# matpalm/cartpoleplusplus

Hardware: AMD Instinct MI355X
Metric: DDPG training steps/sec, 64x64x18 pixel obs, batch=256 (higher is better)
Workload: dtype f32-acc/f16x2,bf16x6

## Files before the change

cartpoleplusplus_amd/csrc/conv3_bwd_pair.hip:

```cpp
#include <cstring>
#ifndef PAIR_ORDER_DEFAULT
#define PAIR_ORDER_DEFAULT 1
#endif
#include "conv_impl.h"
#include "conv_kyo.h"
#include "conv_dx_rs.h"
#include "conv_dw_rs.h"

__global__ __launch_bounds__(CONV_THREADS, 2) void conv3_bwd_pair_kernel(const ConvArgsN dx, int dx_gx, const ConvArgsN dw, int dw_gx, int order) {
  int i;
  if (!pair_grid_place((int)blockIdx.x, dx_gx * dx.n, dw_gx * dw.n, order, &i)) {
    conv_fwd_kyo_body<10, 3, 1, 4, IN_DY, 16, false>(dx, i % dx_gx, i / dx_gx);
  } else {
    conv_dw_body<10, 3, 1, IN_F32_PLAIN>(dw, i % dw_gx, i / dw_gx, dw_gx);
  }
}

template <int ORDER>
__global__ __launch_bounds__(CONV_THREADS, 2) __attribute__((amdgpu_waves_per_eu(2, 2))) void conv3_bwd_pair_rs_kernel(const ConvArgsN dx, int dx_gx, const ConvArgsN dw, int dw_gx, int upi, int band, int order) {
  int i;
  if (!pair_grid_place((int)blockIdx.x, dx_gx * dx.n, dw_gx * dw.n, order, &i)) {
    conv_dx_rs_body<3, 1, ORDER>(dx, i % dx_gx, i / dx_gx);
  } else {
    conv_dw_rs_body<3, ORDER>(dw, upi, band, i % dw_gx, i / dw_gx);
  }
}

template <int ORDER, bool DXRS>
__global__ __launch_bounds__(CONV_THREADS, 2) void conv3_bwd_pair_mixed_kernel(const ConvArgsN dx, int dx_gx, const ConvArgsN dw, int dw_gx, int upi, int band, int order) {
  int i;
  if (!pair_grid_place((int)blockIdx.x, dx_gx * dx.n, dw_gx * dw.n, order, &i)) {
    if (DXRS) conv_dx_rs_body<3, 1, ORDER>(dx, i % dx_gx, i / dx_gx);
    else conv_fwd_kyo_body<10, 3, 1, 4, IN_DY, 16, false>(dx, i % dx_gx, i / dx_gx);
  } else {
    if (DXRS) conv_dw_body<10, 3, 1, IN_F32_PLAIN>(dw, i % dw_gx, i / dw_gx, dw_gx);
    else conv_dw_rs_body<3, ORDER>(dw, upi, band, i % dw_gx, i / dw_gx);
  }
}

int launch_conv3_bwd_pair(cpp_ctx* ctx, const ConvPairSlot& slot) {
  const bool dx_rs = slot.have_dx && slot.dx_rs, dw_rs = slot.have_dw && slot.dw_rs;
  if (slot.have_dx && slot.have_dw && dx_rs != dw_rs) {
    const bool nine = b16_order(ctx) == B16_NINE;
    auto kern = dx_rs ? (nine ? conv3_bwd_pair_mixed_kernel<B16_NINE, true> : conv3_bwd_pair_mixed_kernel<B16_SIX, true>)
                      : (nine ? conv3_bwd_pair_mixed_kernel<B16_NINE, false> : conv3_bwd_pair_mixed_kernel<B16_SIX, false>);
    const size_t lds = slot.dx_lds > slot.dw_lds ? slot.dx_lds : slot.dw_lds;
    HIP_CHECK(hipFuncSetAttribute((const void*)kern, hipFuncAttributeMaxDynamicSharedMemorySize, (int)lds));
    static const int order = cpp_switch_int("CPP_PAIR3_ORDER", 1);
    prof_begin(ctx);
    hipLaunchKernelGGL(kern, dim3(slot.dx_gx * slot.dx.n + slot.dw_gx * slot.dw.n), dim3(CONV_THREADS), lds, ctx->stream, slot.dx, slot.dx_gx, slot.dw, slot.dw_gx,
                       slot.upi, slot.band, order);
    LAUNCH_CHECK();
    prof_end(ctx, K_CONV3_BWD);
    return 0;
  }
  if (dx_rs || dw_rs) {
    if (!(dx_rs && dw_rs)) { cpp_set_error("conv3 backward pair: one half is missing beside a row-streaming body"); return 1; }
    const bool nine = b16_order(ctx) == B16_NINE;
    auto kern = nine ? conv3_bwd_pair_rs_kernel<B16_NINE> : conv3_bwd_pair_rs_kernel<B16_SIX>;
    const size_t lds = slot.dx_lds > slot.dw_lds ? slot.dx_lds : slot.dw_lds;
    static bool attr_done[CPP_MAX_DEVICES][2] = {};
    if (!attr_done[cpp_dev_slot(ctx)][nine ? 1 : 0]) {
      HIP_CHECK(hipFuncSetAttribute((const void*)kern, hipFuncAttributeMaxDynamicSharedMemorySize, (int)lds));
      attr_done[cpp_dev_slot(ctx)][nine ? 1 : 0] = true;
    }
    static const int order = cpp_switch_int("CPP_PAIR3_ORDER", 1);
    prof_begin(ctx);
    hipLaunchKernelGGL(kern, dim3(slot.dx_gx * slot.dx.n + slot.dw_gx * slot.dw.n), dim3(CONV_THREADS), lds, ctx->stream, slot.dx, slot.dx_gx, slot.dw, slot.dw_gx,
                       slot.upi, slot.band, order);
    LAUNCH_CHECK();
    prof_end(ctx, K_CONV3_BWD);
    return 0;
  }
  const int ndx = slot.have_dx ? slot.dx_gx * slot.dx.n : 0, ndw = slot.have_dw ? slot.dw_gx * slot.dw.n : 0;
  if (ndx + ndw == 0) return 0;
  const size_t lds = (slot.have_dx ? slot.dx_lds : 0) > (slot.have_dw ? slot.dw_lds : 0) ? slot.dx_lds : slot.dw_lds;
  static size_t attr_dev[CPP_MAX_DEVICES] = {};
  size_t& attr = attr_dev[cpp_dev_slot(ctx)];
  if (lds > attr) {
    HIP_CHECK(hipFuncSetAttribute((const void*)conv3_bwd_pair_kernel, hipFuncAttributeMaxDynamicSharedMemorySize, (int)lds));
    attr = lds;
  }
  ConvArgsN dx = slot.dx, dw = slot.dw;
  if (!slot.have_dx) { memset(&dx, 0, sizeof(dx)); dx.n = 0; }
  if (!slot.have_dw) { memset(&dw, 0, sizeof(dw)); dw.n = 0; }
  static const int order = cpp_switch_int("CPP_PAIR_ORDER", PAIR_ORDER_DEFAULT);
  prof_begin(ctx);
  hipLaunchKernelGGL(conv3_bwd_pair_kernel, dim3(ndx + ndw), dim3(CONV_THREADS), lds, ctx->stream, dx, slot.have_dx ? slot.dx_gx : 1,
                     dw, slot.have_dw ? slot.dw_gx : 1, order);
  LAUNCH_CHECK();
  prof_end(ctx, K_CONV3_BWD);
  return 0;
}
```

cartpoleplusplus_amd/csrc/conv_dw_rs.hip:

```cpp
#include <cstring>
#include "conv_dw_rs.h"

int conv_dw_rs_dispatch(cpp_ctx* ctx, int cin, int ks, int in_mode, const ConvArgsN& batch, int* grid_out, bool* handled) {
  *handled = false;
  static const bool off = cpp_switch_off("CPP_CONV_DWRS") || cpp_switch_off("CPP_CONV_B16");
  const ConvArgs& a = batch.a[0];
  static const bool off3 = cpp_switch_off("CPP_CONV3_DWRS");
  static const bool w16 = cpp_switch_int("CPP_CONV3_DWRS_W16", 0) != 0;
  const bool geo5 = ks == 5 && (a.W == 32 || a.W == 64), geo3 = ks == 3 && !off3 && ((a.W == 16 && (w16 || conv3_pair_rs_ok(ctx, a.H, a.W))) || a.W == 32 || a.W == 64);
  if (off || !(geo5 || geo3) || cin != KYO_NO || in_mode != IN_F32_PLAIN || (a.H & 1) || a.H < 8 || a.nout != KYO_NO) return 0;
  for (int i = 0; i < batch.n; ++i)
    if (batch.a[i].dy_dense != nullptr || ((uintptr_t)batch.a[i].in & 7) || (batch.a[i].in_bstride & 1)) return 0;
  *handled = true;
  const int capacity = ctx->num_cus * 4 / batch.n, ncol = (a.W + 31) / 32;
  int band = (a.H + 1) & ~1;
  while (band > 8 && (band / 2) % 2 == 0 && a.B * ncol * ((a.H + band / 2 - 1) / (band / 2)) <= capacity) band /= 2;
  const int upi = ((a.H + band - 1) / band) * ncol;
  const int grid = (a.B * upi + 3) / 4;
  if ((size_t)grid > (size_t)ctx->num_cus * 4) { *handled = false; return 0; }
  *grid_out = grid;
  const bool nine = b16_order(ctx) == B16_NINE;
  if (ctx->pair && ctx->pair->layer == 1 && ks == 5 && a.W == 32) {
    ctx->pair->dw = batch; ctx->pair->dw_gx = grid; ctx->pair->dw_lds = DwRsGeom<5>::LDS_BYTES; ctx->pair->have_dw = true;
    ctx->pair->upi = upi; ctx->pair->band = band; ctx->pair->dw_rs = true;
    return 0;
  }
  if (ks == 3 && conv3_pair_rs_ok(ctx, a.H, a.W)) {
    ctx->pair->dw = batch; ctx->pair->dw_gx = grid; ctx->pair->dw_lds = DwRsGeom<3>::LDS_BYTES; ctx->pair->have_dw = true;
    ctx->pair->upi = upi; ctx->pair->band = band; ctx->pair->dw_rs = true;
    return 0;
  }
  typedef void (*kern_t)(const ConvArgsN, int, int);
  const kern_t kern = ks == 5 ? (nine ? (kern_t)conv_dw_rs_kernel<5, B16_NINE> : (kern_t)conv_dw_rs_kernel<5, B16_SIX>)
                              : (nine ? (kern_t)conv_dw_rs_kernel<3, B16_NINE> : (kern_t)conv_dw_rs_kernel<3, B16_SIX>);
  const int lds = ks == 5 ? DwRsGeom<5>::LDS_BYTES : DwRsGeom<3>::LDS_BYTES;
  static bool attr_done[CPP_MAX_DEVICES][4] = {};
  bool& done = attr_done[cpp_dev_slot(ctx)][(nine ? 1 : 0) + (ks == 5 ? 0 : 2)];
  if (!done) {
    HIP_CHECK(hipFuncSetAttribute((const void*)kern, hipFuncAttributeMaxDynamicSharedMemorySize, lds));
    done = true;
  }
  hipLaunchKernelGGL(kern, dim3(grid, batch.n), dim3(CONV_THREADS), lds, ctx->stream, batch, upi, band);
  LAUNCH_CHECK();
  return 0;
}
```

cartpoleplusplus_amd/csrc/conv_dx_rs.h:

```cpp
#pragma once
#include <type_traits>
#include "conv_k16.h"

typedef unsigned dxrs_u32x2 __attribute__((ext_vector_type(2)));

template <int KS_, int TPR>
struct DxRsGeom {
  static constexpr int KS = KS_, P = KS / 2, CH = KYO_NO, NCH = (KS * CH + 31) / 32, NSET = KS + 1;
  static constexpr int UNR = KS == 5 ? 6 : 12;
  static constexpr int W = 16 * TPR, IPW = 4 / TPR;
  static constexpr int NW = KS * KS * CH * CH;
  static constexpr int AIMG_BYTES = KS * NCH * 3 * 1024;
  static constexpr int WPX = 16 + 2 * P;
  static constexpr int PLB = ((2 * CH * 15 + 64 * (NCH - 1) + 64 + 15) & ~15) + 16;
  static constexpr int SLOTB = 3 * PLB;
  static constexpr int TRB = 640 + 16;
  static constexpr int WVB = 2 * SLOTB + TRB;
  static constexpr int LDS_BYTES = AIMG_BYTES + 4 * WVB;
  static_assert((KS == 5 || KS == 3) && 4 % TPR == 0 && WVB % 16 == 0 && PLB >= 2 * CH * WPX + 8, "geometry");
};

template <int KSZ, int TPR, int ORDER>
__device__ __forceinline__ void conv_dx_rs_body(const ConvArgsN& batch, const int bx, const int by) {
  typedef DxRsGeom<KSZ, TPR> G;
  constexpr int KS = G::KS, P = G::P, CH = G::CH, NCH = G::NCH, NSET = G::NSET, UNR = G::UNR, W = G::W, Wp = W / 2;
  constexpr int PLB = G::PLB, SLOTB = G::SLOTB;
  const ConvArgs& a = batch.a[by];
  extern __shared__ __attribute__((aligned(16))) unsigned char dxrs_lds[];
  const int tid = threadIdx.x, lane = tid & 63, li = lane & 15, lj = lane >> 4;
  const int swave = __builtin_amdgcn_readfirstlane(tid >> 6);
  const int simg = swave / TPR, stile = swave % TPR;
  const int nbands = a.nbands > 1 ? a.nbands : 1;
  const int band = bx % nbands;
  const int sb = (bx / nbands) * G::IPW + simg;
  const int H = a.H, Hp = H >> 1;
  const int ylo = nbands > 1 ? band * a.band_rows : 0, yhi = nbands > 1 ? min(H, ylo + a.band_rows) : H;
  const int qbeg = ((ylo > P ? ylo - P : 0) / UNR) * UNR;
  const int qmf = min(H, yhi + P);
  unsigned char* wvb = dxrs_lds + G::AIMG_BYTES + swave * G::WVB;
  constexpr unsigned BIG = 0x08000000u;
  const int cw = lane / 5, op = lane - cw * 5;
  const int ppx = stile * 8 - 1 + cw;
  const bool cell = lane < 50 && ppx >= 0 && ppx < Wp && sb < a.B;
  const __amdgpu_buffer_rsrc_t dp_rsrc = __builtin_amdgcn_make_buffer_rsrc(const_cast<float*>(a.dy.dpool + (long)(sb < a.B ? sb : 0) * a.dy.dpool_bstride), 0,
                                                                           Hp * Wp * CH * 4, 0x00020000);
  const __amdgpu_buffer_rsrc_t am_rsrc = __builtin_amdgcn_make_buffer_rsrc(const_cast<uint8_t*>(a.dy.amax + (long)(sb < a.B ? sb : 0) * Hp * Wp * CH), 0,
                                                                           Hp * Wp * CH, 0x00020000);
  const unsigned goff = cell ? (unsigned)((ppx * CH + 2 * op) * 4) : BIG;
  const unsigned coff = cell ? (unsigned)(ppx * CH + 2 * op) : BIG;
  constexpr int DUMP = PLB - 8;
  const int pe = 2 * cw - 2 + P, po = pe + 1;
  const uint32_t sadr_e = keep_in_vgpr(lds_addr(wvb + ((lane < 50 && pe >= 0 && pe < G::WPX) ? 2 * CH * pe + 4 * op : DUMP)));
  const uint32_t sadr_o = keep_in_vgpr(lds_addr(wvb + ((lane < 50 && po >= 0 && po < G::WPX) ? 2 * CH * po + 4 * op : DUMP)));
  f32x2 rawg[3] = {{0.f, 0.f}, {0.f, 0.f}, {0.f, 0.f}};
  unsigned rawc[3] = {0u, 0u, 0u};
  unsigned pk[3] = {0u, 0u, 0u};
  unsigned mk[2][2] = {{0u, 0u}, {0u, 0u}};
  auto load_pooled = [&](const int buf, const int py) __attribute__((always_inline)) {
    const bool in = py < Hp;
    const dxrs_u32x2 g = __builtin_amdgcn_raw_buffer_load_b64(dp_rsrc, (int)(in ? goff + (unsigned)(py * (Wp * CH * 4)) : BIG), 0, 0);
    rawg[buf] = (f32x2){__uint_as_float(g.x), __uint_as_float(g.y)};
    rawc[buf] = (unsigned)(unsigned short)__builtin_amdgcn_raw_buffer_load_b16(am_rsrc, (int)(in ? coff + (unsigned)(py * (Wp * CH)) : BIG), 0, 0);
  };
  load_pooled(0, qbeg >> 1);
  load_pooled(1, (qbeg >> 1) + 1);
  unsigned char* aimg = dxrs_lds;
  {
    constexpr int NWT = (G::NW + CONV_THREADS - 1) / CONV_THREADS;
    float wr[NWT];
#pragma unroll
    for (int n = 0; n < NWT; ++n) { const int i = tid + n * CONV_THREADS; wr[n] = a.w[i < G::NW ? i : 0]; }
    for (int i = tid; i < G::AIMG_BYTES / 16; i += CONV_THREADS) reinterpret_cast<k16_u32x4*>(aimg)[i] = (k16_u32x4){0u, 0u, 0u, 0u};
    for (int i = lane; i < G::WVB / 16; i += 64) reinterpret_cast<k16_u32x4*>(wvb)[i] = (k16_u32x4){0u, 0u, 0u, 0u};
    __syncthreads();
#pragma unroll
    for (int n = 0; n < NWT; ++n) {
      const int i = tid + n * CONV_THREADS;
      if (i < G::NW) {
        const int o = i % CH, c = (i / CH) % CH, t = i / (CH * CH), kx = t % KS, ky = t / KS;
        const int k = (KS - 1 - kx) * CH + o, ch = k >> 5, lg = (k >> 3) & 3, e = k & 7;
        unsigned short h, m, l;
        k16_split3(a.wscale != 0.f ? wr[n] * a.wscale : wr[n], h, m, l);
        unsigned short* d = reinterpret_cast<unsigned short*>(aimg + (((KS - 1 - ky) * NCH + ch) * 3) * 1024 + (lg * 16 + c) * 16 + e * 2);
        d[0] = h; d[512] = m; d[1024] = l;
      }
    }
  }
  __syncthreads();
  if (sb >= a.B) return;
  k16_u32x4 wv[KS][NCH][3];
#pragma unroll
  for (int ky = 0; ky < KS; ++ky)
#pragma unroll
    for (int ch = 0; ch < NCH; ++ch)
#pragma unroll
      for (int pc = 0; pc < 3; ++pc)
        wv[ky][ch][pc] = *reinterpret_cast<const k16_u32x4*>(aimg + ((ky * NCH + ch) * 3 + pc) * 1024 + lane * 16);

  auto convert = [&](const int buf) __attribute__((always_inline)) {
    const unsigned c0 = rawc[buf] & 0xFFu, c1 = rawc[buf] >> 8;
    const float g0 = (c0 & POOL_ACTIVE) ? rawg[buf][0] : 0.f, g1 = (c1 & POOL_ACTIVE) ? rawg[buf][1] : 0.f;
    unsigned short h0, m0, l0, h1, m1, l1;
    k16_split3(g0, h0, m0, l0); k16_split3(g1, h1, m1, l1);
    pk[0] = (unsigned)h0 | ((unsigned)h1 << 16); pk[1] = (unsigned)m0 | ((unsigned)m1 << 16); pk[2] = (unsigned)l0 | ((unsigned)l1 << 16);
    const unsigned p0 = c0 & 3u, p1 = c1 & 3u;
#pragma unroll
    for (int ry = 0; ry < 2; ++ry)
#pragma unroll
      for (int rx = 0; rx < 2; ++rx)
        mk[ry][rx] = (p0 == (unsigned)(2 * ry + rx) ? 0xFFFFu : 0u) | (p1 == (unsigned)(2 * ry + rx) ? 0xFFFF0000u : 0u);
  };
  auto stage_row = [&](const int slot, const int ry) __attribute__((always_inline)) {
#pragma unroll
    for (int p = 0; p < 3; ++p) {
      lds_store(sadr_e, slot * SLOTB + p * PLB, pk[p] & mk[ry][0]);
      lds_store(sadr_o, slot * SLOTB + p * PLB, pk[p] & mk[ry][1]);
    }
  };
  const uint32_t xrd = keep_in_vgpr(lds_addr(wvb + 2 * CH * li + 16 * lj));
  k16_u32x4 xb[NCH][3];
  auto read_x = [&](const int ch, const int slot) __attribute__((always_inline)) {
#pragma unroll
    for (int p = 0; p < 3; ++p) {
      unsigned t[4];
#pragma unroll
      for (int i = 0; i < 4; ++i) t[i] = lds_load<unsigned>(xrd, slot * SLOTB + p * PLB + 64 * ch + 4 * i);
      xb[ch][p] = (k16_u32x4){t[0], t[1], t[2], t[3]};
    }
  };

  const __amdgpu_buffer_rsrc_t out_rsrc = __builtin_amdgcn_make_buffer_rsrc(a.out + (long)sb * a.out_bstride, 0, H * W * CH * 4, 0x00020000);
  unsigned char* trw = wvb + 2 * SLOTB;
  const uint32_t twA = keep_in_vgpr(lds_addr(trw + (lj < 3 ? (li * CH + 4 * lj) * 4 : 640)));
  const uint32_t twB = keep_in_vgpr(lds_addr(trw + (lj < 2 ? (li * CH + 4 * lj + 2) * 4 : 648)));
  const uint32_t trd = keep_in_vgpr(lds_addr(trw + (lane < 4 * CH ? 16 * lane : 0)));
  const unsigned eL = lane < 4 * CH ? (unsigned)(stile * 16 * CH * 4 + 16 * lane) : BIG;

  f32x4 acc[NSET];
#pragma unroll
  for (int s = 0; s < NSET; ++s) acc[s] = (f32x4){0.f, 0.f, 0.f, 0.f};
  const f32x4 zero4 = {0.f, 0.f, 0.f, 0.f};
  float vmx = 0.f;

  convert(0);
  stage_row(0, 0);
  read_x(0, 0);
  if (NCH > 1) read_x(NCH - 1, 0);
  __builtin_amdgcn_sched_barrier(0);

  auto step = [&](auto sqtag, auto gentag, const int q) __attribute__((always_inline)) {
    constexpr int SQ = decltype(sqtag)::value;
    constexpr bool GEN = decltype(gentag)::value;
    constexpr int SD = (SQ + 2 * NSET - P - 1) % NSET;
    constexpr int SLOT = SQ & 1;
    constexpr bool EVEN = (SQ & 1) == 0;
    const int yd = q - P - 1;
    auto epi_write = [&]() __attribute__((always_inline)) {
      lds_store(twA, 0, (f32x2){acc[SD][0], acc[SD][1]});
      lds_store(twB, 0, (f32x2){acc[SD][2], acc[SD][3]});
    };
    auto epi_store = [&]() __attribute__((always_inline)) {
      const f32x4 v = lds_load<f32x4>(trd, 0);
      const bool live = !GEN || (yd >= ylo && yd < yhi);
      if (KS == 5) {
        const float m = fmaxf(fmaxf(fabsf(v[0]), fabsf(v[1])), fmaxf(fabsf(v[2]), fabsf(v[3])));
        vmx = fmaxf(vmx, live ? m : 0.f);
      }
      buffer_store_b128_held((k16_u32x4){__float_as_uint(v[0]), __float_as_uint(v[1]), __float_as_uint(v[2]), __float_as_uint(v[3])},
                             out_rsrc, (int)(live ? eL : BIG), (live ? yd : 0) * (W * CH * 4));
    };
    auto mfmas = [&](auto chtag) __attribute__((always_inline)) {
      constexpr int ch = decltype(chtag)::value;
#pragma unroll
      for (int sum = ORDER; sum >= 0; --sum)
#pragma unroll
        for (int pa = 2; pa >= 0; --pa) {
          const int pb = sum - pa;
          if (pb >= 0 && pb <= 2) {
#pragma unroll
            for (int ky = 0; ky < KS; ++ky) {
              const int s = (SQ + P - ky + NSET) % NSET;
              const bool restart = ch == 0 && sum == ORDER && pa == 2 && ky == 0;
              acc[s] = __builtin_amdgcn_mfma_f32_16x16x32_bf16(__builtin_bit_cast(k16_bf16x8, wv[ky][ch][pa]), __builtin_bit_cast(k16_bf16x8, xb[ch][pb]),
                                                               restart ? zero4 : acc[s], 0, 0, 0);
            }
          }
        }
    };
    constexpr int J = (SQ / 2) % 3;
    if (!GEN || q < qmf) {
      constexpr int NMF = (ORDER == B16_NINE ? 9 : 6) * KS;
      if constexpr (NCH == 1) {
        mfmas(std::integral_constant<int, 0>{});
        stage_row(SLOT ^ 1, EVEN ? 1 : 0);
        if (EVEN) load_pooled((J + 2) % 3, (q >> 1) + 2);
        epi_write();
        read_x(0, SLOT ^ 1);
        epi_store();
        if (EVEN) convert((J + 1) % 3);
        __builtin_amdgcn_sched_barrier(0);
      } else {
      mfmas(std::integral_constant<int, 0>{});
      stage_row(SLOT ^ 1, EVEN ? 1 : 0);
      if (EVEN) load_pooled((J + 2) % 3, (q >> 1) + 2);
      epi_write();
      read_x(0, SLOT ^ 1);
#pragma unroll
      for (int i = 0; i < NMF; ++i) {
        __builtin_amdgcn_sched_group_barrier(0x008, 1, 0);
        if (i < 4) __builtin_amdgcn_sched_group_barrier(0x002, 3, 0);
        else if (i < 9) __builtin_amdgcn_sched_group_barrier(0x200, 1, 0);
        else if (i < 15) __builtin_amdgcn_sched_group_barrier(0x100, 1, 0);
        if (EVEN && i == 4) __builtin_amdgcn_sched_group_barrier(0x020, 2, 0);
      }
      __builtin_amdgcn_sched_barrier(0);
      mfmas(std::integral_constant<int, 1>{});
      epi_store();
      if (EVEN) convert((J + 1) % 3);
      read_x(1, SLOT ^ 1);
#pragma unroll
      for (int i = 0; i < NMF; ++i) {
        __builtin_amdgcn_sched_group_barrier(0x008, 1, 0);
        if (i == 0) __builtin_amdgcn_sched_group_barrier(0x100, 1, 0);
        else if (i == 4) __builtin_amdgcn_sched_group_barrier(0x040, 1, 0);
        else if (EVEN && i < NMF - 3) __builtin_amdgcn_sched_group_barrier(0x002, 2, 0);
        else if (i >= NMF - 3) __builtin_amdgcn_sched_group_barrier(0x100, 2, 0);
      }
      __builtin_amdgcn_sched_barrier(0);
      }
    } else { epi_write(); epi_store(); }
  };
  auto block = [&](auto gentag, const int q0) __attribute__((always_inline)) {
    constexpr bool GEN = decltype(gentag)::value;
    const int qe = yhi + P + 1;
    if (GEN && q0 + 0 >= qe) return; step(std::integral_constant<int, 0>{}, gentag, q0 + 0);
    if (GEN && q0 + 1 >= qe) return; step(std::integral_constant<int, 1>{}, gentag, q0 + 1);
    if (GEN && q0 + 2 >= qe) return; step(std::integral_constant<int, 2>{}, gentag, q0 + 2);
    if (GEN && q0 + 3 >= qe) return; step(std::integral_constant<int, 3>{}, gentag, q0 + 3);
    if (GEN && q0 + 4 >= qe) return; step(std::integral_constant<int, 4>{}, gentag, q0 + 4);
    if (GEN && q0 + 5 >= qe) return; step(std::integral_constant<int, 5>{}, gentag, q0 + 5);
    if constexpr (UNR == 12) {
      if (GEN && q0 + 6 >= qe) return; step(std::integral_constant<int, 6>{}, gentag, q0 + 6);
      if (GEN && q0 + 7 >= qe) return; step(std::integral_constant<int, 7>{}, gentag, q0 + 7);
      if (GEN && q0 + 8 >= qe) return; step(std::integral_constant<int, 8>{}, gentag, q0 + 8);
      if (GEN && q0 + 9 >= qe) return; step(std::integral_constant<int, 9>{}, gentag, q0 + 9);
      if (GEN && q0 + 10 >= qe) return; step(std::integral_constant<int, 10>{}, gentag, q0 + 10);
      if (GEN && q0 + 11 >= qe) return; step(std::integral_constant<int, 11>{}, gentag, q0 + 11);
    }
  };
  int q0 = qbeg;
  block(std::true_type{}, q0); q0 += UNR;
  for (; q0 >= ylo + P + 1 && q0 + UNR <= qmf; q0 += UNR) block(std::false_type{}, q0);
  for (; q0 < yhi + P + 1; q0 += UNR) block(std::true_type{}, q0);
  if (KS == 5 && a.dx_imax) {
    for (int o = 32; o > 0; o >>= 1) vmx = fmaxf(vmx, __shfl_xor(vmx, o));
    if (lane == 0 && sb < a.B) {
      float* im = a.dx_imax + (long)sb * DX_IMAX_SLOTS;
      for (int t = stile; t < 4; t += TPR) {
        if (nbands > 1) im[2 * t + band] = vmx; else { im[2 * t] = vmx; im[2 * t + 1] = vmx; }
      }
    }
  }
}

template <int KSZ, int TPR, int ORDER>
__global__ __launch_bounds__(CONV_THREADS, 2) __attribute__((amdgpu_waves_per_eu(2, 2))) void conv_dx_rs_kernel(const ConvArgsN batch) {
  conv_dx_rs_body<KSZ, TPR, ORDER>(batch, blockIdx.x, blockIdx.y);
}

int conv_dx_rs_dispatch(cpp_ctx* ctx, int cin, int ks, int in_mode, const ConvArgsN& a, bool* handled);
bool conv_dx_rs_ok(const cpp_ctx* ctx, int cin, int ks, int H, int W, int nout);
```

cartpoleplusplus_amd/csrc/conv_dx_rs.hip:

```cpp
#include <cstring>
#include "conv_dx_rs.h"

template <int KS, int TPR, int ORDER>
static int conv_dx_rs_launch_t(cpp_ctx* ctx, const ConvArgsN& batch) {
  typedef DxRsGeom<KS, TPR> G;
  const ConvArgs& a = batch.a[0];
  auto kern = conv_dx_rs_kernel<KS, TPR, ORDER>;
  static bool attr_done[CPP_MAX_DEVICES] = {};
  if (!attr_done[cpp_dev_slot(ctx)]) {
    HIP_CHECK(hipFuncSetAttribute((const void*)kern, hipFuncAttributeMaxDynamicSharedMemorySize, G::LDS_BYTES));
    attr_done[cpp_dev_slot(ctx)] = true;
  }
  const int nb = a.nbands > 1 ? a.nbands : 1;
  hipLaunchKernelGGL(kern, dim3(((a.B + G::IPW - 1) / G::IPW) * nb, batch.n), dim3(CONV_THREADS), G::LDS_BYTES, ctx->stream, batch);
  LAUNCH_CHECK();
  return 0;
}

bool conv3_pair_rs_ok(const cpp_ctx* ctx, int H, int W) {
  static const bool off = cpp_switch_off("CPP_CONV3_PAIR_RS") || cpp_switch_off("CPP_CONV_DXRS") || cpp_switch_off("CPP_CONV_DWRS") ||
                          cpp_switch_off("CPP_CONV3_DXRS") || cpp_switch_off("CPP_CONV3_DWRS") || cpp_switch_off("CPP_CONV_B16") || cpp_switch_off("CPP_CONV3_PAIR");
  return !off && ctx && ctx->pair && ctx->pair->layer == 2 && W == 16 && H >= 8 && !(H & 1);
}

bool conv_dx_rs_ok(const cpp_ctx* ctx, int cin, int ks, int H, int W, int nout) {
  static const bool off = cpp_switch_off("CPP_CONV_DXRS") || cpp_switch_off("CPP_CONV_B16") || cpp_switch_off("CPP_CONV_KYO");
  (void)ctx;
  static const bool off3 = cpp_switch_off("CPP_CONV3_DXRS");
  static const bool w16 = cpp_switch_int("CPP_CONV3_DXRS_W16", 0) != 0;
  const bool geo = (ks == 5 && (W == 32 || W == 64)) || (ks == 3 && !off3 && ((W == 16 && (w16 || conv3_pair_rs_ok(ctx, H, W))) || W == 32 || W == 64));
  return !off && cin == KYO_NO && nout == KYO_NO && geo && H >= 4 && !(H & 1);
}

int conv_dx_rs_dispatch(cpp_ctx* ctx, int cin, int ks, int in_mode, const ConvArgsN& a_in, bool* handled) {
  *handled = false;
  const ConvArgs& a0 = a_in.a[0];
  if (in_mode != IN_DY || !conv_dx_rs_ok(ctx, cin, ks, a0.H, a0.W, a0.nout)) return 0;
  *handled = true;
  const bool nine = b16_order(ctx) == B16_NINE;
  ConvArgsN a = a_in;
  {
    static const int bands_sw = cpp_switch_int("CPP_DXRS_BANDS", 1);
    const int ipw = a0.W == 16 ? 4 : (a0.W == 32 ? 2 : 1);
    const int wgs = a.n * ((a0.B + ipw - 1) / ipw);
    const bool paired = (ctx->pair && ctx->pair->layer == 1 && a0.W == 32) || (ks == 3 && conv3_pair_rs_ok(ctx, a0.H, a0.W));
    const bool two = bands_sw != 0 && ((wgs < ctx->num_cus && !paired) || bands_sw == 2) && a0.H >= 16 && (a0.H % 4) == 0;
    for (int i = 0; i < a.n; ++i) { a.a[i].nbands = two ? 2 : 1; a.a[i].band_rows = two ? a0.H / 2 : a0.H; }
  }
  if (ctx->pair && ctx->pair->layer == 1 && ks == 5 && a0.W == 32) {
    ctx->pair->dx = a; ctx->pair->dx_gx = ((a0.B + 1) / 2) * a.a[0].nbands; ctx->pair->dx_lds = DxRsGeom<5, 2>::LDS_BYTES; ctx->pair->have_dx = true;
    ctx->pair->dx_rs = true;
    return 0;
  }
  if (ks == 3 && conv3_pair_rs_ok(ctx, a0.H, a0.W) && a0.nout == KYO_NO) {
    ctx->pair->dx = a; ctx->pair->dx_gx = ((a0.B + 3) / 4) * a.a[0].nbands; ctx->pair->dx_lds = DxRsGeom<3, 1>::LDS_BYTES; ctx->pair->have_dx = true;
    ctx->pair->dx_rs = true;
    return 0;
  }
  if (ks == 3) {
    if (a0.W == 16) return nine ? conv_dx_rs_launch_t<3, 1, B16_NINE>(ctx, a) : conv_dx_rs_launch_t<3, 1, B16_SIX>(ctx, a);
    if (a0.W == 32) return nine ? conv_dx_rs_launch_t<3, 2, B16_NINE>(ctx, a) : conv_dx_rs_launch_t<3, 2, B16_SIX>(ctx, a);
    return nine ? conv_dx_rs_launch_t<3, 4, B16_NINE>(ctx, a) : conv_dx_rs_launch_t<3, 4, B16_SIX>(ctx, a);
  }
  if (a0.W == 32) return nine ? conv_dx_rs_launch_t<5, 2, B16_NINE>(ctx, a) : conv_dx_rs_launch_t<5, 2, B16_SIX>(ctx, a);
  return nine ? conv_dx_rs_launch_t<5, 4, B16_NINE>(ctx, a) : conv_dx_rs_launch_t<5, 4, B16_SIX>(ctx, a);
}
```

Baseline: 3157.

## Add two-row-per-trip dW body for conv3 pair and band dX when it fits

Adds a new row-streaming weight-gradient body for the 3x3, 16-wide layer. Each trip processes two input rows against pooled dy rows, using a ring of staged input and gradient slots in LDS and 16x16x32 bf16 MFMAs. It is enabled by default in the paired backward kernel. The dX side of that pair now splits into two row bands when twice the workgroup count still fits on the CUs, and its band start is aligned to 6 rather than the unroll size, so the first block skips the leading steps. The new kernel adds a larger LDS footprint and a complex pipeline, which could limit occupancy or add risk at the band edges.

New measurement: 3167 (median of 3 runs). About the same (+0.3%).

```diff
diff --git a/cartpoleplusplus_amd/csrc/conv3_bwd_pair.hip b/cartpoleplusplus_amd/csrc/conv3_bwd_pair.hip
--- a/cartpoleplusplus_amd/csrc/conv3_bwd_pair.hip
+++ b/cartpoleplusplus_amd/csrc/conv3_bwd_pair.hip
@@ -6,6 +6,7 @@
 #include "conv_kyo.h"
 #include "conv_dx_rs.h"
 #include "conv_dw_rs.h"
+#include "conv_dw_rs2.h"
 
 __global__ __launch_bounds__(CONV_THREADS, 2) void conv3_bwd_pair_kernel(const ConvArgsN dx, int dx_gx, const ConvArgsN dw, int dw_gx, int order) {
   int i;
@@ -16,13 +17,14 @@
   }
 }
 
-template <int ORDER>
+template <int ORDER, bool ROWS2>
 __global__ __launch_bounds__(CONV_THREADS, 2) __attribute__((amdgpu_waves_per_eu(2, 2))) void conv3_bwd_pair_rs_kernel(const ConvArgsN dx, int dx_gx, const ConvArgsN dw, int dw_gx, int upi, int band, int order) {
   int i;
   if (!pair_grid_place((int)blockIdx.x, dx_gx * dx.n, dw_gx * dw.n, order, &i)) {
     conv_dx_rs_body<3, 1, ORDER>(dx, i % dx_gx, i / dx_gx);
   } else {
-    conv_dw_rs_body<3, ORDER>(dw, upi, band, i % dw_gx, i / dw_gx);
+    if (ROWS2) conv_dw_rs2_body<ORDER>(dw, upi, band, i % dw_gx, i / dw_gx);
+    else conv_dw_rs_body<3, ORDER>(dw, upi, band, i % dw_gx, i / dw_gx);
   }
 }
 
@@ -57,8 +59,11 @@
   if (dx_rs || dw_rs) {
     if (!(dx_rs && dw_rs)) { cpp_set_error("conv3 backward pair: one half is missing beside a row-streaming body"); return 1; }
     const bool nine = b16_order(ctx) == B16_NINE;
-    auto kern = nine ? conv3_bwd_pair_rs_kernel<B16_NINE> : conv3_bwd_pair_rs_kernel<B16_SIX>;
-    const size_t lds = slot.dx_lds > slot.dw_lds ? slot.dx_lds : slot.dw_lds;
+    static const bool rows2 = cpp_switch_int("CPP_CONV3_DW_ROWS2", 1) != 0;
+    auto kern = rows2 ? (nine ? conv3_bwd_pair_rs_kernel<B16_NINE, true> : conv3_bwd_pair_rs_kernel<B16_SIX, true>)
+                      : (nine ? conv3_bwd_pair_rs_kernel<B16_NINE, false> : conv3_bwd_pair_rs_kernel<B16_SIX, false>);
+    const size_t dw_lds = rows2 ? (size_t)DwRs2Geom::LDS_BYTES : slot.dw_lds;
+    const size_t lds = slot.dx_lds > dw_lds ? slot.dx_lds : dw_lds;
     static bool attr_done[CPP_MAX_DEVICES][2] = {};
     if (!attr_done[cpp_dev_slot(ctx)][nine ? 1 : 0]) {
       HIP_CHECK(hipFuncSetAttribute((const void*)kern, hipFuncAttributeMaxDynamicSharedMemorySize, (int)lds));
diff --git a/cartpoleplusplus_amd/csrc/conv_dw_rs.hip b/cartpoleplusplus_amd/csrc/conv_dw_rs.hip
--- a/cartpoleplusplus_amd/csrc/conv_dw_rs.hip
+++ b/cartpoleplusplus_amd/csrc/conv_dw_rs.hip
@@ -15,6 +15,8 @@
   const int capacity = ctx->num_cus * 4 / batch.n, ncol = (a.W + 31) / 32;
   int band = (a.H + 1) & ~1;
   while (band > 8 && (band / 2) % 2 == 0 && a.B * ncol * ((a.H + band / 2 - 1) / (band / 2)) <= capacity) band /= 2;
+  static const int band3_sw = cpp_switch_int("CPP_CONV3_DW_BAND", 0);
+  if (ks == 3 && (band3_sw == 4 || band3_sw == 8 || band3_sw == 16) && band3_sw <= ((a.H + 1) & ~1)) band = band3_sw;
   const int upi = ((a.H + band - 1) / band) * ncol;
   const int grid = (a.B * upi + 3) / 4;
   if ((size_t)grid > (size_t)ctx->num_cus * 4) { *handled = false; return 0; }
diff --git a/cartpoleplusplus_amd/csrc/conv_dw_rs2.h b/cartpoleplusplus_amd/csrc/conv_dw_rs2.h
--- /dev/null
+++ b/cartpoleplusplus_amd/csrc/conv_dw_rs2.h
@@ -0,0 +1,247 @@
+#pragma once
+#include "conv_dw_rs.h"
+
+struct DwRs2Geom {
+  static constexpr int KS = 3, P = 1, PB = 2, CIN = KYO_NO, NO = KYO_NO, W = 16, CP = 12, MT = 3, NT = 2;
+  static constexpr int WPX = W + 2 * P;
+  static constexpr int ROWB = 2 * (((CP * WPX + 16 * MT - KS * CP) + 7) & ~7);
+  static constexpr int XSLOT = 3 * ROWB, XPAIR = 2 * XSLOT;
+  static constexpr int NXP = 2;
+  static constexpr int DOST = 48, DPC = NO * DOST;
+  static constexpr int DSLOT = 3 * DPC;
+  static constexpr int NDS = 8;
+  static constexpr int WVB = NXP * XPAIR + NDS * DSLOT;
+  static constexpr int LDS_BYTES = 4 * WVB;
+  static constexpr int UNR = 12;
+  static_assert(ROWB % 16 == 0 && WVB % 16 == 0 && WVB >= MT * NT * 4 * 64 * 4, "the wave's slots also hold its accumulators for the final sum");
+  static_assert(LDS_BYTES <= 80 * 1024, "two workgroups per CU");
+  static_assert(2 * NXP * W == 64, "one lane per ones-channel pixel");
+};
+
+template <int ORDER>
+__device__ __forceinline__ void conv_dw_rs2_body(const ConvArgsN& batch, const int units_per_img, const int band, const int bx, const int by) {
+  typedef DwRs2Geom G;
+  constexpr int KS = G::KS, P = G::P, PB = G::PB, CIN = G::CIN, NO = G::NO, W = G::W, Wp = W / 2, CP = G::CP, MT = G::MT, NT = G::NT;
+  constexpr int ROWB = G::ROWB, XSLOT = G::XSLOT, XPAIR = G::XPAIR, DOST = G::DOST, DPC = G::DPC, DSLOT = G::DSLOT, NDS = G::NDS;
+  constexpr unsigned BIG = 0x08000000u;
+  const ConvArgs& a = batch.a[by];
+  extern __shared__ __attribute__((aligned(16))) unsigned char dwrs_lds[];
+  const int tid = threadIdx.x, lane = tid & 63, li = lane & 15, lj = lane >> 4;
+  const int swave = __builtin_amdgcn_readfirstlane(tid >> 6);
+  unsigned char* wvb = dwrs_lds + swave * G::WVB;
+  unsigned char* xring = wvb;
+  unsigned char* dzring = wvb + G::NXP * XPAIR;
+  const int H = a.H, Hp = H >> 1;
+  const int units = a.B * units_per_img;
+  const int unit = bx * 4 + swave;
+  const bool work = unit < units;
+  const int ub = work ? unit / units_per_img : 0;
+  const int uin = unit - ub * units_per_img;
+  const int q_lo = work ? uin * band : 0;
+  const int rows = work ? min(band, H - q_lo) : 0;
+  const int y0 = q_lo - PB;
+
+  for (int i = lane; i < G::WVB / 16; i += 64) reinterpret_cast<k16_u32x4*>(wvb)[i] = (k16_u32x4){0u, 0u, 0u, 0u};
+  *reinterpret_cast<unsigned short*>(xring + (lane >> 4) * XSLOT + 2 * (CP * ((lane & 15) + P) + CIN)) = (unsigned short)0x3F80u;
+
+  constexpr int NXV = 3;
+  const __amdgpu_buffer_rsrc_t in_rsrc = __builtin_amdgcn_make_buffer_rsrc(
+      const_cast<float*>((const float*)a.in + (long)ub * a.in_bstride), 0, work ? H * W * CIN * 4 : 0, 0x00020000);
+  unsigned xvo[NXV]; uint32_t xdst[NXV];
+#pragma unroll
+  for (int i = 0; i < NXV; ++i) {
+    const int idx = lane + 64 * i, r = idx / (5 * G::WPX), rem = idx - r * (5 * G::WPX), wx = rem / 5, cp = rem - 5 * wx;
+    const int x = wx - P;
+    const bool on = idx < 2 * 5 * G::WPX;
+    xvo[i] = (on && x >= 0 && x < W) ? (unsigned)(r * (W * CIN * 4) + 8 * (5 * x + cp)) : BIG;
+    xdst[i] = keep_in_vgpr(lds_addr(xring + (on ? r * XSLOT + 2 * (CP * wx + 2 * cp) : ROWB - 8)));
+  }
+  f32x2 xraw[2][NXV];
+  auto x_load = [&](const int buf, const int q) __attribute__((always_inline)) {
+    const unsigned ro = q < H ? (unsigned)(q * (W * CIN * 4)) : BIG;
+#pragma unroll
+    for (int i = 0; i < NXV; ++i) {
+      const dw16_u32x2 v = __builtin_amdgcn_raw_buffer_load_b64(in_rsrc, (int)(xvo[i] + ro), 0, 0);
+      xraw[buf][i] = (f32x2){__uint_as_float(v.x), __uint_as_float(v.y)};
+    }
+  };
+  auto x_store = [&](const int buf, const int ps) __attribute__((always_inline)) {
+#pragma unroll
+    for (int i = 0; i < NXV; ++i) {
+      unsigned short h0, m0, l0, h1, m1, l1;
+      dwb_split3(xraw[buf][i][0], h0, m0, l0); dwb_split3(xraw[buf][i][1], h1, m1, l1);
+      lds_store(xdst[i], ps * XPAIR, (unsigned)h0 | ((unsigned)h1 << 16));
+      lds_store(xdst[i], ps * XPAIR + ROWB, (unsigned)m0 | ((unsigned)m1 << 16));
+      lds_store(xdst[i], ps * XPAIR + 2 * ROWB, (unsigned)l0 | ((unsigned)l1 << 16));
+    }
+  };
+
+  const int zg = lane / NO, zo = lane - zg * NO;
+  const bool zon = lane < 2 * NO;
+  const __amdgpu_buffer_rsrc_t dp_rsrc = __builtin_amdgcn_make_buffer_rsrc(const_cast<float*>(a.dy.dpool + (long)ub * a.dy.dpool_bstride), 0,
+                                                                           work ? Hp * Wp * NO * 4 : 0, 0x00020000);
+  const __amdgpu_buffer_rsrc_t am_rsrc = __builtin_amdgcn_make_buffer_rsrc(const_cast<uint8_t*>(a.dy.amax + (long)ub * Hp * Wp * NO), 0,
+                                                                           work ? Hp * Wp * NO : 0, 0x00020000);
+  const unsigned zoff = zon ? (unsigned)(zg * NO + zo) : BIG;
+  const uint32_t zdst = keep_in_vgpr(lds_addr(dzring + (zon ? zo * DOST + zg * 16 : DOST - 16)));
+  float zrg[3][4]; unsigned zrc[3][4];
+#pragma unroll
+  for (int b = 0; b < 3; ++b)
+#pragma unroll
+    for (int j = 0; j < 4; ++j) { zrg[b][j] = 0.f; zrc[b][j] = 0u; }
+  unsigned zp01[3] = {0u, 0u, 0u}, zp23[3] = {0u, 0u, 0u};
+  unsigned zm01[4] = {0u, 0u, 0u, 0u}, zm23[4] = {0u, 0u, 0u, 0u};
+  auto z_load = [&](const int buf, const int py) __attribute__((always_inline)) {
+    const unsigned ro = (py >= 0 && py < Hp) ? (unsigned)(py * (Wp * NO)) : BIG;
+#pragma unroll
+    for (int j = 0; j < 4; ++j) {
+      const unsigned e = zoff + ro + (unsigned)(2 * j * NO);
+      zrg[buf][j] = __uint_as_float(__builtin_amdgcn_raw_buffer_load_b32(dp_rsrc, (int)(e * 4u), 0, 0));
+      zrc[buf][j] = (unsigned)__builtin_amdgcn_raw_buffer_load_b8(am_rsrc, (int)e, 0, 0);
+    }
+  };
+  auto z_convert = [&](const int buf) __attribute__((always_inline)) {
+#pragma unroll
+    for (int hf = 0; hf < 2; ++hf) {
+      unsigned short pc[2][3];
+#pragma unroll
+      for (int j = 0; j < 2; ++j) {
+        const float g = (zrc[buf][2 * hf + j] & POOL_ACTIVE) ? zrg[buf][2 * hf + j] : 0.f;
+        dwb_split3(g, pc[j][0], pc[j][1], pc[j][2]);
+      }
+#pragma unroll
+      for (int p = 0; p < 3; ++p) {
+        const unsigned v = (unsigned)pc[0][p] | ((unsigned)pc[1][p] << 16);
+        if (hf == 0) zp01[p] = v; else zp23[p] = v;
+      }
+#pragma unroll
+      for (int pos = 0; pos < 4; ++pos) {
+        const unsigned v = ((zrc[buf][2 * hf] & 3u) == (unsigned)pos ? 0xFFFFu : 0u) | ((zrc[buf][2 * hf + 1] & 3u) == (unsigned)pos ? 0xFFFF0000u : 0u);
+        if (hf == 0) zm01[pos] = v; else zm23[pos] = v;
+      }
+    }
+  };
+  auto z_store = [&](const int slot, const int ry) __attribute__((always_inline)) {
+#pragma unroll
+    for (int p = 0; p < 3; ++p)
+      lds_store(zdst, slot * DSLOT + p * DPC, (k16_u32x4){zp01[p] & zm01[2 * ry], zp23[p] & zm23[2 * ry], zp01[p] & zm01[2 * ry + 1], zp23[p] & zm23[2 * ry + 1]});
+  };
+
+  const int tj = (lane >> 2) & 3, tq = lane & 3;
+  const uint32_t aadr = keep_in_vgpr(lds_addr(xring + (lj & 1) * XSLOT + 2 * (CP * (4 * tj + 2 * (lj >> 1)) + 4 * tq)));
+  uint32_t bbase[NT]; int brk[NT];
+#pragma unroll
+  for (int nt = 0; nt < NT; ++nt) {
+    const int n = 16 * nt + li;
+    const bool nvalid = n < KS * NO;
+    brk[nt] = (lj & 1) - (nvalid ? n / NO : 0) + P + PB;
+    bbase[nt] = lds_addr(dzring + (nvalid ? n % NO : 0) * DOST + (lj >> 1) * 16);
+  }
+  f32x4 acc[MT][NT];
+#pragma unroll
+  for (int mt = 0; mt < MT; ++mt)
+#pragma unroll
+    for (int nt = 0; nt < NT; ++nt) acc[mt][nt] = (f32x4){0.f, 0.f, 0.f, 0.f};
+
+  if (work) {
+    const int py0 = y0 >> 1;
+    z_load(0, py0); z_load(1, py0 + 1); z_load(2, py0 + 2);
+    x_load(0, q_lo); x_load(1, q_lo + 2);
+#pragma unroll
+    for (int d = 0; d < 3; ++d) { z_convert(d); z_store(2 * d, 0); z_store(2 * d + 1, 1); }
+    z_load(0, py0 + 3); z_load(1, py0 + 4); z_load(2, py0 + 5);
+    x_store(0, 0);
+    x_load(0, q_lo + 4);
+    __builtin_amdgcn_sched_barrier(0);
+
+    k16_u32x4 bq[NT][3];
+    k16_u32x4 av[3];
+    auto trip = [&](auto tqtag, const int T) __attribute__((always_inline)) {
+      constexpr int TQ = decltype(tqtag)::value;
+      constexpr int XS = TQ & 1, ZBUF = TQ % 3, ZSL = (2 * TQ + 6) % NDS;
+#pragma unroll
+      for (int nt = 0; nt < NT; ++nt) {
+        const int sl = ((2 * TQ) % NDS + brk[nt]) & (NDS - 1);
+        const uint32_t ad = bbase[nt] + (uint32_t)(sl * DSLOT);
+#pragma unroll
+        for (int p = 0; p < 3; ++p) bq[nt][p] = lds_load<k16_u32x4>(ad, p * DPC);
+      }
+#pragma unroll
+      for (int mt = 0; mt < MT; ++mt) {
+#pragma unroll
+        for (int pa = 0; pa < 3; ++pa) {
+          const int off = XS * XPAIR + pa * ROWB + mt * 32;
+          const dw16_v4s r0 = __builtin_amdgcn_ds_read_tr16_b64_v4i16(
+              reinterpret_cast<__attribute__((address_space(3))) dw16_v4s*>((uintptr_t)(aadr + (uint32_t)off)));
+          const dw16_v4s r1 = __builtin_amdgcn_ds_read_tr16_b64_v4i16(
+              reinterpret_cast<__attribute__((address_space(3))) dw16_v4s*>((uintptr_t)(aadr + (uint32_t)(off + 2 * CP))));
+          const dw16_u32x2 u0 = __builtin_bit_cast(dw16_u32x2, r0), u1 = __builtin_bit_cast(dw16_u32x2, r1);
+          av[pa] = (k16_u32x4){u0.x, u0.y, u1.x, u1.y};
+        }
+#pragma unroll
+        for (int sum = ORDER; sum >= 0; --sum)
+#pragma unroll
+          for (int pa = 2; pa >= 0; --pa) {
+            const int pb = sum - pa;
+            if (pb >= 0 && pb <= 2) {
+#pragma unroll
+              for (int nt = 0; nt < NT; ++nt)
+                acc[mt][nt] = __builtin_amdgcn_mfma_f32_16x16x32_bf16(__builtin_bit_cast(dwb_bf16x8, av[pa]), __builtin_bit_cast(dwb_bf16x8, bq[nt][pb]),
+                                                                      acc[mt][nt], 0, 0, 0);
+            }
+          }
+        if (mt == 0) z_convert(ZBUF);
+        else if (mt == 1) { z_store(ZSL, 0); z_store(ZSL + 1, 1); z_load(ZBUF, py0 + T + 6); }
+        else { x_store((TQ + 1) & 1, XS ^ 1); x_load((TQ + 1) & 1, q_lo + 2 * T + 6); }
+      }
+      __builtin_amdgcn_sched_barrier(0);
+    };
+    const int ntrips = rows >> 1;
+    for (int T0 = 0; T0 < ntrips; T0 += G::UNR) {
+      if (T0 + 0 < ntrips) trip(std::integral_constant<int, 0>{}, T0 + 0);
+      if (T0 + 1 < ntrips) trip(std::integral_constant<int, 1>{}, T0 + 1);
+      if (T0 + 2 < ntrips) trip(std::integral_constant<int, 2>{}, T0 + 2);
+      if (T0 + 3 < ntrips) trip(std::integral_constant<int, 3>{}, T0 + 3);
+      if (T0 + 4 < ntrips) trip(std::integral_constant<int, 4>{}, T0 + 4);
+      if (T0 + 5 < ntrips) trip(std::integral_constant<int, 5>{}, T0 + 5);
+      if (T0 + 6 < ntrips) trip(std::integral_constant<int, 6>{}, T0 + 6);
+      if (T0 + 7 < ntrips) trip(std::integral_constant<int, 7>{}, T0 + 7);
+      if (T0 + 8 < ntrips) trip(std::integral_constant<int, 8>{}, T0 + 8);
+      if (T0 + 9 < ntrips) trip(std::integral_constant<int, 9>{}, T0 + 9);
+      if (T0 + 10 < ntrips) trip(std::integral_constant<int, 10>{}, T0 + 10);
+      if (T0 + 11 < ntrips) trip(std::integral_constant<int, 11>{}, T0 + 11);
+    }
+  }
+
+  float* mine = reinterpret_cast<float*>(wvb);
+#pragma unroll
+  for (int mt = 0; mt < MT; ++mt)
+#pragma unroll
+    for (int nt = 0; nt < NT; ++nt)
+      *reinterpret_cast<f32x4*>(mine + ((mt * NT + nt) * 64 + lane) * 4) = acc[mt][nt];
+  __syncthreads();
+  float* part = a.partial + (long)bx * a.pstride;
+#pragma unroll
+  for (int tile = 0; tile < MT * NT; ++tile) {
+    if ((tile & 3) != swave) continue;
+    const int mt = tile / NT, nt = tile - mt * NT;
+    const int n = 16 * nt + li;
+    const bool nvalid = n < KS * NO;
+    const int nky = nvalid ? n / NO : 0, no = nvalid ? n % NO : 0;
+    f32x4 s = *reinterpret_cast<const f32x4*>(reinterpret_cast<const float*>(dwrs_lds) + (tile * 64 + lane) * 4);
+#pragma unroll
+    for (int v = 1; v < 4; ++v) {
+      const f32x4 o = *reinterpret_cast<const f32x4*>(reinterpret_cast<const float*>(dwrs_lds + v * G::WVB) + (tile * 64 + lane) * 4);
+      s[0] += o[0]; s[1] += o[1]; s[2] += o[2]; s[3] += o[3];
+    }
+    if (nvalid && no < a.nout) {
+#pragma unroll
+      for (int r = 0; r < 4; ++r) {
+        const int m = 16 * mt + 4 * lj + r;
+        const int kx = m / CP, c = m - kx * CP;
+        if (kx < KS && c < CIN) part[(nky * (KS * CIN) + kx * CIN + c) * a.nout + no] = s[r];
+        else if (kx == P && c == CIN && nky == P) part[DwRsGeom<3>::NW / NO * a.nout + no] = s[r];
+      }
+    }
+  }
+}
diff --git a/cartpoleplusplus_amd/csrc/conv_dx_rs.h b/cartpoleplusplus_amd/csrc/conv_dx_rs.h
--- a/cartpoleplusplus_amd/csrc/conv_dx_rs.h
+++ b/cartpoleplusplus_amd/csrc/conv_dx_rs.h
@@ -35,7 +35,7 @@
   const int sb = (bx / nbands) * G::IPW + simg;
   const int H = a.H, Hp = H >> 1;
   const int ylo = nbands > 1 ? band * a.band_rows : 0, yhi = nbands > 1 ? min(H, ylo + a.band_rows) : H;
-  const int qbeg = ((ylo > P ? ylo - P : 0) / UNR) * UNR;
+  const int qbeg = ((ylo > P ? ylo - P : 0) / 6) * 6;
   const int qmf = min(H, yhi + P);
   unsigned char* wvb = dxrs_lds + G::AIMG_BYTES + swave * G::WVB;
   constexpr unsigned BIG = 0x08000000u;
@@ -233,12 +233,13 @@
   auto block = [&](auto gentag, const int q0) __attribute__((always_inline)) {
     constexpr bool GEN = decltype(gentag)::value;
     const int qe = yhi + P + 1;
-    if (GEN && q0 + 0 >= qe) return; step(std::integral_constant<int, 0>{}, gentag, q0 + 0);
-    if (GEN && q0 + 1 >= qe) return; step(std::integral_constant<int, 1>{}, gentag, q0 + 1);
-    if (GEN && q0 + 2 >= qe) return; step(std::integral_constant<int, 2>{}, gentag, q0 + 2);
-    if (GEN && q0 + 3 >= qe) return; step(std::integral_constant<int, 3>{}, gentag, q0 + 3);
-    if (GEN && q0 + 4 >= qe) return; step(std::integral_constant<int, 4>{}, gentag, q0 + 4);
-    if (GEN && q0 + 5 >= qe) return; step(std::integral_constant<int, 5>{}, gentag, q0 + 5);
+    const bool mid = GEN && UNR == 12 && q0 < qbeg;
+    if (GEN && q0 + 0 >= qe) return; if (!mid) step(std::integral_constant<int, 0>{}, gentag, q0 + 0);
+    if (GEN && q0 + 1 >= qe) return; if (!mid) step(std::integral_constant<int, 1>{}, gentag, q0 + 1);
+    if (GEN && q0 + 2 >= qe) return; if (!mid) step(std::integral_constant<int, 2>{}, gentag, q0 + 2);
+    if (GEN && q0 + 3 >= qe) return; if (!mid) step(std::integral_constant<int, 3>{}, gentag, q0 + 3);
+    if (GEN && q0 + 4 >= qe) return; if (!mid) step(std::integral_constant<int, 4>{}, gentag, q0 + 4);
+    if (GEN && q0 + 5 >= qe) return; if (!mid) step(std::integral_constant<int, 5>{}, gentag, q0 + 5);
     if constexpr (UNR == 12) {
       if (GEN && q0 + 6 >= qe) return; step(std::integral_constant<int, 6>{}, gentag, q0 + 6);
       if (GEN && q0 + 7 >= qe) return; step(std::integral_constant<int, 7>{}, gentag, q0 + 7);
@@ -248,7 +249,7 @@
       if (GEN && q0 + 11 >= qe) return; step(std::integral_constant<int, 11>{}, gentag, q0 + 11);
     }
   };
-  int q0 = qbeg;
+  int q0 = UNR == 6 ? qbeg : (qbeg / UNR) * UNR;
   block(std::true_type{}, q0); q0 += UNR;
   for (; q0 >= ylo + P + 1 && q0 + UNR <= qmf; q0 += UNR) block(std::false_type{}, q0);
   for (; q0 < yhi + P + 1; q0 += UNR) block(std::true_type{}, q0);
diff --git a/cartpoleplusplus_amd/csrc/conv_dx_rs.hip b/cartpoleplusplus_amd/csrc/conv_dx_rs.hip
--- a/cartpoleplusplus_amd/csrc/conv_dx_rs.hip
+++ b/cartpoleplusplus_amd/csrc/conv_dx_rs.hip
@@ -43,8 +43,10 @@
     static const int bands_sw = cpp_switch_int("CPP_DXRS_BANDS", 1);
     const int ipw = a0.W == 16 ? 4 : (a0.W == 32 ? 2 : 1);
     const int wgs = a.n * ((a0.B + ipw - 1) / ipw);
-    const bool paired = (ctx->pair && ctx->pair->layer == 1 && a0.W == 32) || (ks == 3 && conv3_pair_rs_ok(ctx, a0.H, a0.W));
-    const bool two = bands_sw != 0 && ((wgs < ctx->num_cus && !paired) || bands_sw == 2) && a0.H >= 16 && (a0.H % 4) == 0;
+    const bool pair2 = ctx->pair && ctx->pair->layer == 1 && a0.W == 32, pair3 = ks == 3 && conv3_pair_rs_ok(ctx, a0.H, a0.W);
+    static const int bands3_sw = cpp_switch_int("CPP_CONV3_PAIR_BANDS", 1);
+    const bool fits = pair3 ? (bands3_sw != 0 && 2 * wgs <= ctx->num_cus) : (wgs < ctx->num_cus && !pair2);
+    const bool two = bands_sw != 0 && (fits || bands_sw == 2) && a0.H >= 16 && (a0.H % 4) == 0;
     for (int i = 0; i < a.n; ++i) { a.a[i].nbands = two ? 2 : 1; a.a[i].band_rows = two ? a0.H / 2 : a0.H; }
   }
   if (ctx->pair && ctx->pair->layer == 1 && ks == 5 && a0.W == 32) {
```
